# filrg/split_learning

Hardware: AMD Instinct MI355X
Metric: images/sec (whole node) VGG16/CIFAR10 cut=7 (higher is better)
Workload: dtype fp32; 1 GPU; model=VGG16_CIFAR10, global_batch=32, image=3x32x32, cut_layer=7, optimizer=SGD(lr=5e-4, momentum=0.5), control_count=1, mode=serial-recompute, parallelism=split2 x dp1

## Files before the change

split_learning_amd/ops/csrc/bindings.cpp:

```cpp
#include <torch/extension.h>

namespace slk {
at::Tensor matmul_f32(const at::Tensor&, const at::Tensor&, bool, bool,
                      c10::optional<at::Tensor>, bool);
at::Tensor linear_fwd(const at::Tensor&, const at::Tensor&, c10::optional<at::Tensor>);
at::Tensor colsum_f32(const at::Tensor&);
at::Tensor conv2d_wino(const at::Tensor&, const at::Tensor&,
                       c10::optional<at::Tensor>, int, bool);
int conv2d_wino_slabs(int, int, int);
at::Tensor conv2d_wino_bwdw(const at::Tensor&, const at::Tensor&, int);
at::Tensor conv2d_wino_fused(const at::Tensor&, const at::Tensor&,
                             c10::optional<at::Tensor>, int, bool);
at::Tensor conv2d_wino_bwdw_fused(const at::Tensor&, const at::Tensor&, int);
at::Tensor conv2d_fwd(const at::Tensor&, const at::Tensor&, c10::optional<at::Tensor>,
                      int, int);
at::Tensor conv2d_bwd_data(const at::Tensor&, const at::Tensor&, int, int, int, int);
at::Tensor conv2d_bwd_weight(const at::Tensor&, const at::Tensor&, int, int, int, int);
at::Tensor conv2d_bwd_bias(const at::Tensor&);
std::string conv_route(const std::string&, int, int, int, int, int, int, int, int);
std::vector<at::Tensor> bn2d_stats_fused(const at::Tensor&,
                                         c10::optional<at::Tensor>,
                                         c10::optional<at::Tensor>,
                                         c10::optional<at::Tensor>, double, double);
at::Tensor bn2d_fwd(const at::Tensor&, const at::Tensor&, const at::Tensor&,
                    const at::Tensor&, const at::Tensor&, bool);
std::vector<at::Tensor> bn2d_bwd(const at::Tensor&, const at::Tensor&,
                                 const at::Tensor&, const at::Tensor&,
                                 const at::Tensor&, c10::optional<at::Tensor>);
std::vector<at::Tensor> bn2d_bwd_eval(const at::Tensor&, const at::Tensor&,
                                      const at::Tensor&, const at::Tensor&,
                                      const at::Tensor&, c10::optional<at::Tensor>);
std::vector<at::Tensor> bn2d_train_fwd(const at::Tensor&, const at::Tensor&,
                                       const at::Tensor&,
                                       c10::optional<at::Tensor>,
                                       c10::optional<at::Tensor>,
                                       c10::optional<at::Tensor>, double, double,
                                       bool, bool);
std::vector<at::Tensor> bn2d_train_bwd(const at::Tensor&, const at::Tensor&,
                                       const at::Tensor&, const at::Tensor&,
                                       const at::Tensor&, c10::optional<at::Tensor>,
                                       c10::optional<at::Tensor>);
std::vector<at::Tensor> drop_res_ln_fwd(const at::Tensor&, const at::Tensor&,
                                        const at::Tensor&, const at::Tensor&,
                                        double, double, int64_t,
                                        c10::optional<at::Tensor>);
std::vector<at::Tensor> layernorm_fwd(const at::Tensor&, const at::Tensor&,
// ... 36 lines not shown
                double, double, double, double, bool);
at::Tensor make_opt_desc(std::vector<at::Tensor>, std::vector<at::Tensor>,
                         std::vector<at::Tensor>, std::vector<at::Tensor>);
void sgd_step_fused(const at::Tensor&, int64_t, int64_t, double, double, double,
                    bool, bool);
void adamw_step_fused(const at::Tensor&, int64_t, int64_t, int64_t, double, double,
                      double, double, double, bool);
}

PYBIND11_MODULE(TORCH_EXTENSION_NAME, m) {
  m.doc() = "split_learning_amd CDNA4 (gfx950) HIP kernels";
  m.def("matmul_f32", &slk::matmul_f32, py::arg("a"), py::arg("b"),
        py::arg("trans_a") = false, py::arg("trans_b") = false,
        py::arg("out") = py::none(), py::arg("accumulate") = false);
  m.def("linear_fwd", &slk::linear_fwd);
  m.def("colsum_f32", &slk::colsum_f32);
  m.def("conv2d_wino", &slk::conv2d_wino, py::arg("x"), py::arg("w"),
        py::arg("bias") = py::none(), py::arg("pad") = 1,
        py::arg("flip") = false);
  m.def("conv2d_wino_slabs", &slk::conv2d_wino_slabs, py::arg("co"),
        py::arg("ci"), py::arg("tiles"));
  m.def("conv2d_wino_bwdw", &slk::conv2d_wino_bwdw, py::arg("gy"),
        py::arg("x"), py::arg("pad") = 1);
  m.def("conv2d_wino_fused", &slk::conv2d_wino_fused, py::arg("x"),
        py::arg("w"), py::arg("bias") = py::none(), py::arg("pad") = 1,
        py::arg("flip") = false);
  m.def("conv2d_wino_bwdw_fused", &slk::conv2d_wino_bwdw_fused, py::arg("gy"),
        py::arg("x"), py::arg("pad") = 1);
  m.def("conv2d_fwd", &slk::conv2d_fwd, py::arg("x"), py::arg("w"),
        py::arg("bias"), py::arg("stride"), py::arg("pad"));
  m.def("conv2d_bwd_data", &slk::conv2d_bwd_data);
  m.def("conv2d_bwd_weight", &slk::conv2d_bwd_weight, py::arg("gy"), py::arg("x"),
        py::arg("kh"), py::arg("kw"), py::arg("stride"), py::arg("pad"));
  m.def("conv2d_bwd_bias", &slk::conv2d_bwd_bias);
  m.def("conv_route", &slk::conv_route, py::arg("op"), py::arg("B"),
        py::arg("Ci"), py::arg("H"), py::arg("W"), py::arg("Co"), py::arg("K"),
        py::arg("stride"), py::arg("pad"));
  m.def("bn2d_stats_fused", &slk::bn2d_stats_fused);
  m.def("bn2d_fwd", &slk::bn2d_fwd);
  m.def("bn2d_bwd", &slk::bn2d_bwd, py::arg("x"), py::arg("gy"),
        py::arg("gamma"), py::arg("mean"), py::arg("invstd"),
        py::arg("relu_y") = py::none());
  m.def("bn2d_bwd_eval", &slk::bn2d_bwd_eval, py::arg("x"), py::arg("gy"),
        py::arg("gamma"), py::arg("mean"), py::arg("invstd"),
        py::arg("relu_y") = py::none());
  m.def("bn2d_train_fwd", &slk::bn2d_train_fwd, py::arg("x"), py::arg("gamma"),
        py::arg("beta"), py::arg("running_mean"), py::arg("running_var"),
        py::arg("num_batches_tracked"), py::arg("momentum"), py::arg("eps"),
        py::arg("relu") = false, py::arg("pool") = false);
  m.def("bn2d_train_bwd", &slk::bn2d_train_bwd, py::arg("x"), py::arg("gy"),
        py::arg("gamma"), py::arg("mean"), py::arg("invstd"),
        py::arg("relu_y") = py::none(), py::arg("idx") = py::none());
  m.def("drop_res_ln_fwd", &slk::drop_res_ln_fwd, py::arg("x"), py::arg("res"),
        py::arg("gamma"), py::arg("beta"), py::arg("eps"), py::arg("p") = 0.0,
        py::arg("seed") = 0, py::arg("offset") = py::none());
  m.def("layernorm_fwd", &slk::layernorm_fwd);
  m.def("layernorm_bwd", &slk::layernorm_bwd);
  m.def("relu_fwd", &slk::relu_fwd);
  m.def("relu_bwd", &slk::relu_bwd);
  m.def("gelu_fwd", &slk::gelu_fwd);
  m.def("gelu_bwd", &slk::gelu_bwd);
  m.def("tanh_fwd", &slk::tanh_fwd);
  m.def("tanh_bwd", &slk::tanh_bwd);
  m.def("dropout_fwd", &slk::dropout_fwd);
  m.def("dropout_fwd_dev", &slk::dropout_fwd_dev);
  m.def("dropout_bwd", &slk::dropout_bwd);
// ... 25 lines not shown
```

split_learning_amd/ops/csrc/conv2d.hip:

```cpp
#include <tuple>

#include "conv_route.h"
#include "tile_gemm.h"
#include "torch_util.h"

namespace slk {

at::Tensor conv2d_wino(const at::Tensor&, const at::Tensor&,
                       c10::optional<at::Tensor>, int, bool);
at::Tensor conv2d_wino_bwdw(const at::Tensor&, const at::Tensor&, int);
at::Tensor conv2d_wino_fused(const at::Tensor&, const at::Tensor&,
                             c10::optional<at::Tensor>, int, bool);
at::Tensor conv2d_wino_bwdw_fused(const at::Tensor&, const at::Tensor&, int);

static int wino_level() {
  static const int v = [] {
    const char* e = std::getenv("SLK_WINO");
    return e ? atoi(e) : 1;
  }();
  return v;
}

struct ConvGeom {
  int B, Ci, H, W, Co, KH, KW, OH, OW, stride, pad;
  FastDiv d_ohow, d_ow, d_hw, d_w, d_khkw, d_kw;
};

template <int CKH, int CKW, int CS>
struct Geo {
  static constexpr bool fixed = CKH > 0;
  __device__ static int kh_kw(const ConvGeom& g) { return fixed ? CKH * CKW : g.KH * g.KW; }
  __device__ static int stride(const ConvGeom& g) { return fixed ? CS : g.stride; }
  __device__ static void dk(const ConvGeom& g, int k, int& c, int& kh, int& kw) {
    if (fixed) {
      c = k / (CKH * CKW);
      const int r = k - c * (CKH * CKW);
      kh = r / CKW;
      kw = r - kh * CKW;
    } else {
      c = g.d_khkw.div(k);
      const int r = g.d_khkw.mod(k, c);
      kh = g.d_kw.div(r);
      kw = g.d_kw.mod(r, kh);
    }
  }
};
// ... 180 lines not shown
    return {ci * geo.H * geo.W, (short)kh, (short)kw, valid};
  }
  __device__ float loadB(const BCtx& c, const KCtx&, int k, bool kv) const {
    const unsigned b = geo.d_ohow.div(k);
    const unsigned rem = geo.d_ohow.mod(k, b);
    const unsigned oh = geo.d_ow.div(rem);
    const unsigned ow = geo.d_ow.mod(rem, oh);
    const int ih = (int)oh * G::stride(geo) - geo.pad + c.kh;
    const int iw = (int)ow * G::stride(geo) - geo.pad + c.kw;
    const bool in = (unsigned)ih < (unsigned)geo.H && (unsigned)iw < (unsigned)geo.W;
    const int ihc = in ? ih : 0;
    const int iwc = in ? iw : 0;
    const float v = x[(long)b * geo.Ci * geo.H * geo.W + c.ciHW
                      + ihc * geo.W + iwc];
    return sel0(v, c.valid & kv & in);
  }
};

struct AtomicStore {
  float* c;
  int N;
  bool accumulate;
  long slab_stride;
  __device__ void store(int, int m, int n, float v, int ks) const {
    float* p = c + (long)ks * slab_stride + (long)m * N + n;
    if (accumulate) {
      atomicAdd(p, v);
    } else {
      *p = v;
    }
  }
};

__global__ void slab_reduce_kernel(const float* __restrict__ slab, int splits,
                                   float* __restrict__ out, long numel) {
  const long stride = (long)gridDim.x * blockDim.x;
  for (long i = (long)blockIdx.x * blockDim.x + threadIdx.x; i < numel;
       i += stride) {
    float s = 0.f;
    for (int k = 0; k < splits; ++k) s += slab[(long)k * numel + i];
    out[i] = s;
  }
}

void slab_reduce(const float* slab, int splits, float* out, long numel,
                 hipStream_t stream) {
  const int grid = (int)std::min<long>((numel + 255) / 256, 4096);
  hipLaunchKernelGGL(slab_reduce_kernel, dim3(grid), dim3(256), 0, stream,
                     slab, splits, out, numel);
}

static inline int slab_min_splits() {
  static int v = [] {
    const char* e = std::getenv("SLK_SLAB_MIN");
    return e ? atoi(e) : 3;
  }();
  return v < 2 ? 2 : v;
}

static constexpr long SLK_SLAB_MAX_BYTES = 32l << 20;


static ConvShape conv_shape(int B, int Ci, int H, int W, int Co, int KH, int KW,
                            int stride, int pad) {
  return {B, Ci, H, W, Co, KH, KW, stride, pad};
}

static ConvGeom make_geom(const ConvShape& s) {
  ConvGeom g;
  g.B = s.B; g.Ci = s.Ci; g.H = s.H; g.W = s.W; g.Co = s.Co; g.KH = s.KH;
  g.KW = s.KW; g.stride = s.stride; g.pad = s.pad;
  g.OH = s.OH();
  g.OW = s.OW();
  g.d_ohow.init(g.OH * g.OW);
  g.d_ow.init(g.OW);
  g.d_hw.init(g.H * g.W);
  g.d_w.init(g.W);
  g.d_khkw.init(g.KH * g.KW);
  g.d_kw.init(g.KW);
  return g;
}

// ... 124 lines not shown
                                slab_stride};
      });
}

at::Tensor conv2d_bwd_weight(const at::Tensor& gy, const at::Tensor& x, int KH,
                             int KW, int stride, int pad) {
  TORCH_CHECK(gy.is_cuda() && x.is_cuda() && gy.scalar_type() == at::kFloat);
  const ConvShape s = conv_shape(x.size(0), x.size(1), x.size(2), x.size(3),
                                 gy.size(1), KH, KW, stride, pad);
  TORCH_CHECK(s.OH() == gy.size(2) && s.OW() == gy.size(3),
              "bwd-weight geometry mismatch");
  switch (route_bwd_weight(s, wino_level())) {
    case ConvRoute::WinoBwdWFused:
      return conv2d_wino_bwdw_fused(gy, x, pad);
    case ConvRoute::WinoBwdW:
      return conv2d_wino_bwdw(gy, x, pad);
    default:
      break;
  }
  auto gyc = gy.contiguous();
  auto xc = x.contiguous();
  const ConvGeom geo = make_geom(s);
  const int N = geo.Ci * KH * KW;
  const bool fast = (geo.OH * geo.OW) % SLK_BK == 0;
  return direct_gemm<ConvBwdWeightGather>(
      geo, geo.Co, N, geo.B * geo.OH * geo.OW, {geo.Co, geo.Ci, KH, KW},
      gy.options(), gyc.data_ptr<float>(), xc.data_ptr<float>(),
      [&](float* gw, bool accumulate, long slab_stride) {
        return AtomicStore{gw, N, accumulate, slab_stride};
      },
      fast);
}

std::string conv_route(const std::string& op, int B, int Ci, int H, int W,
                       int Co, int K, int stride, int pad) {
  const ConvShape s = conv_shape(B, Ci, H, W, Co, K, K, stride, pad);
  if (op == "fwd") return conv_route_name(route_fwd(s, wino_level()));
  if (op == "bwd_data") return conv_route_name(route_bwd_data(s, wino_level()));
  TORCH_CHECK(op == "bwd_weight", "conv_route: op must be fwd, bwd_data or "
              "bwd_weight, got ", op);
  return conv_route_name(route_bwd_weight(s, wino_level()));
}

__global__ void conv_bias_grad_kernel(const float* __restrict__ gy,
                                      float* __restrict__ slab, int B, int C,
                                      int HW) {
  __shared__ float scratch[16];
  const int c = blockIdx.x;
  const int total = B * HW;
  const int per = (total + gridDim.y - 1) / gridDim.y;
  const int lo = blockIdx.y * per;
  const int hi = min(total, lo + per);
  float acc = 0.f;
  for (int i = lo + threadIdx.x; i < hi; i += blockDim.x) {
    const int b = i / HW;
    const int r = i - b * HW;
    acc += gy[((long)b * C + c) * HW + r];
  }
  float total_s = slk_block_sum(acc, scratch);
  if (threadIdx.x == 0) slab[(long)blockIdx.y * C + c] = total_s;
}

__global__ void conv_bias_finalize_kernel(const float* __restrict__ slab,
                                          int chunks, float* __restrict__ gb,
                                          int C) {
  const int c = blockIdx.x * blockDim.x + threadIdx.x;
// ... 24 lines not shown
```

split_learning_amd/ops/csrc/torch_util.h:

```cpp
#pragma once

#include <torch/extension.h>
#include <ATen/ATen.h>
#include <c10/hip/HIPStream.h>

#include "common.h"

namespace slk {

static inline at::Tensor zeroed(at::IntArrayRef sizes, const at::TensorOptions& opt) {
  auto t = at::empty(sizes, opt);
  slk_zero_async(t.data_ptr<float>(), t.numel(),
                 c10::hip::getCurrentHIPStream().stream());
  return t;
}

static inline int reduce_chunks(long per_channel) {
  long c = per_channel / 4096;
  if (c < 1) c = 1;
  if (c > 16) c = 16;
  return (int)c;
}

void slab_reduce(const float* slab, int splits, float* out, long numel,
                 hipStream_t stream);

}
```

split_learning_amd/ops/csrc/wino.hip:

```cpp
#include "torch_util.h"

namespace slk {

template <bool FLIP>
__device__ __forceinline__ void wino_wt_body(const float* __restrict__ w,
                                             float* __restrict__ U, int Cw0,
                                             int Cw1, int block, int nblocks) {
  const long total = (long)Cw0 * Cw1;
  const long tstride = (long)nblocks * blockDim.x;
  for (long e = (long)block * blockDim.x + threadIdx.x; e < 4 * total;
       e += tstride) {
    const int a = (int)(e & 3);
    const long i = e >> 2;
    const int cols = FLIP ? Cw0 : Cw1;
    const int c = (int)(i % cols);
    const int r = (int)(i / cols);
    const int co = FLIP ? c : r;
    const int ci = FLIP ? r : c;
    float t[3];
    #pragma unroll
    for (int b = 0; b < 3; ++b) {
      const float g0 = w[(((long)co * Cw1 + ci) * 3 + (FLIP ? 2 : 0)) * 3 +
                         (FLIP ? 2 - b : b)];
      const float g1 = w[(((long)co * Cw1 + ci) * 3 + 1) * 3 +
                         (FLIP ? 2 - b : b)];
      const float g2 = w[(((long)co * Cw1 + ci) * 3 + (FLIP ? 0 : 2)) * 3 +
                         (FLIP ? 2 - b : b)];
      t[b] = a == 0 ? g0
           : a == 1 ? 0.5f * (g0 + g1 + g2)
           : a == 2 ? 0.5f * (g0 - g1 + g2)
           : g2;
    }
// ... 288 lines not shown
constexpr int WF_RS = 168;
constexpr int WF_OP = 32 * WF_RS;

__device__ __forceinline__ void wino_kstep_mfma(const float* pa,
                                                const float* pb,
                                                f32x4 (&acc)[16]) {
  const f32x4* a0 = reinterpret_cast<const f32x4*>(pa);
  const f32x4* a1 = reinterpret_cast<const f32x4*>(pa + 4 * WF_KS);
  const f32x4* b0 = reinterpret_cast<const f32x4*>(pb);
  const f32x4* b1 = reinterpret_cast<const f32x4*>(pb + 4 * WF_KS);
  f32x4 ra0 = a0[0], rb0 = b0[0], ra1 = a1[0], rb1 = b1[0];
  #pragma unroll
  for (int g = 0; g < 4; ++g) {
    const f32x4 ca0 = ra0, cb0 = rb0, ca1 = ra1, cb1 = rb1;
    if (g < 3) {
      ra0 = a0[g + 1];
      rb0 = b0[g + 1];
      ra1 = a1[g + 1];
      rb1 = b1[g + 1];
    }
    __builtin_amdgcn_sched_barrier(0);
    #pragma unroll
    for (int j = 0; j < 4; ++j)
      acc[g * 4 + j] = __builtin_amdgcn_mfma_f32_16x16x4f32(
          ca0[j], cb0[j], acc[g * 4 + j], 0, 0, 0);
    #pragma unroll
    for (int j = 0; j < 4; ++j)
      acc[g * 4 + j] = __builtin_amdgcn_mfma_f32_16x16x4f32(
          ca1[j], cb1[j], acc[g * 4 + j], 0, 0, 0);
  }
}

template <bool FLIP>
__global__ __launch_bounds__(256, 3) void wino_fused_kernel(
    const float* __restrict__ x, const float* __restrict__ w,
    const float* __restrict__ bias, float* __restrict__ y, int B, int Ci,
    int H, int W, int Co, int OH, int OW, int tH, int tW, int pad,
    int ci_per, int CW, FastDiv d_thw, FastDiv d_tw) {
  const int ci_begin = blockIdx.z * ci_per;
  const int ci_end = min(Ci, ci_begin + ci_per);
  __shared__ __attribute__((aligned(16))) float Ul[WF_OP];
  __shared__ __attribute__((aligned(16))) float Vl[WF_OP];

  const int T = B * tH * tW;
  const int co0 = blockIdx.y * WF_CO;
  const int t0 = blockIdx.x * WF_T;

  const int tid = threadIdx.x;
  const int lane = tid & 63;
  const int wid = tid >> 6;
  const int wco = (wid >> 1) * 16;
  const int wt = (wid & 1) * 16;
  const int frag_r = lane >> 4;
  const int frag_c = lane & 15;

  f32x4 acc[16];
  #pragma unroll
  for (int f = 0; f < 16; ++f) acc[f] = f32x4{};

  const int v_ci = tid >> 5;
  const int v_t = tid & 31;
  const int tg = t0 + v_t;
  const unsigned vb = d_thw.div((unsigned)tg);
  const unsigned vrem = d_thw.mod((unsigned)tg, vb);
  const unsigned vth = d_tw.div(vrem);
  const unsigned vtw = d_tw.mod(vrem, vth);
  const int ih0 = (int)vth * 2 - pad;
  const int iw0 = (int)vtw * 2 - pad;
  const long xplane = ((long)vb * Ci + v_ci) * H * W;
  const int w_co = tid >> 3;
  const int w_ci = tid & 7;

  float d[4][4];
  f32x4 wq0, wq1;
  float w8;

  auto load_regs = [&](int ci0) {
    const float* xp = x + xplane + (long)ci0 * H * W;
    #pragma unroll
// ... 51 lines not shown
    for (int a = 0; a < 4; ++a) {
      const float* t = tr[a];
      up[a] = f32x4{t[0], 0.5f * (t[0] + t[1] + t[2]),
                    0.5f * (t[0] - t[1] + t[2]), t[2]};
    }
  };

  const float* pa = &Ul[(wco + frag_c) * WF_RS + frag_r * WF_KS];
  const float* pb = &Vl[(wt + frag_c) * WF_RS + frag_r * WF_KS];

  load_regs(ci_begin);
  for (int ci0 = ci_begin; ci0 < ci_end; ci0 += WF_CK) {
    store_stage();
    __syncthreads();
    if (ci0 + WF_CK < ci_end) load_regs(ci0 + WF_CK);
    wino_kstep_mfma(pa, pb, acc);
    __syncthreads();
  }

  #pragma unroll
  for (int i = 0; i < 4; ++i) {
    const int co = co0 + wco + frag_r * 4 + i;
    const int t = t0 + wt + frag_c;
    if (co >= Co || t >= T) continue;
    float m[4][4];
    #pragma unroll
    for (int f = 0; f < 16; ++f) m[f >> 2][f & 3] = acc[f][i];
    float u0[4], u1[4];
    #pragma unroll
    for (int bb = 0; bb < 4; ++bb) {
      u0[bb] = m[0][bb] + m[1][bb] + m[2][bb];
      u1[bb] = m[1][bb] - m[2][bb] - m[3][bb];
    }
    const float bv = (bias != nullptr && blockIdx.z == 0) ? bias[co] : 0.f;
    const unsigned b = d_thw.div((unsigned)t);
    const unsigned rem = d_thw.mod((unsigned)t, b);
    const unsigned th = d_tw.div(rem);
    const unsigned tw = d_tw.mod(rem, th);
    float* yp = y + (long)blockIdx.z * B * Co * OH * OW +
                ((long)b * Co + co) * OH * OW + (long)th * 2 * OW + tw * 2;
    const float o00 = u0[0] + u0[1] + u0[2] + bv;
    const float o01 = u0[1] - u0[2] - u0[3] + bv;
    const float o10 = u1[0] + u1[1] + u1[2] + bv;
    const float o11 = u1[1] - u1[2] - u1[3] + bv;
    yp[0] = o00;
    yp[1] = o01;
    yp[OW] = o10;
    yp[OW + 1] = o11;
  }
}

at::Tensor conv2d_wino_bwdw(const at::Tensor& gy, const at::Tensor& x,
                            int pad) {
  TORCH_CHECK(gy.is_cuda() && x.is_cuda() && gy.dim() == 4 && x.dim() == 4);
  auto gyc = gy.contiguous();
  auto xc = x.contiguous();
  const int B = x.size(0), Ci = x.size(1), H = x.size(2), W = x.size(3);
  const int Co = gy.size(1), OH = gy.size(2), OW = gy.size(3);
  TORCH_CHECK(OH == H + 2 * pad - 2 && OW == W + 2 * pad - 2,
              "wino_bwdw geometry");
  TORCH_CHECK(OH % 2 == 0 && OW % 2 == 0, "wino_bwdw: even output dims only");
  const int tH = OH / 2, tW = OW / 2;
  const int T = B * tH * tW;
  auto stream = c10::hip::getCurrentHIPStream().stream();
  FastDiv d_T, d_thw, d_tw;
  d_T.init(T);
  d_thw.init(tH * tW);
  d_tw.init(tW);

  auto Wg = at::empty({16, Co, T}, x.options());
  auto Vx = at::empty({16, Ci, T}, x.options());
  {
    const long tot = (long)Co * T;
    const int grid = (int)std::min<long>((tot + 255) / 256, 8192);
    hipLaunchKernelGGL(wino_gyA_kernel, dim3(grid), dim3(256), 0, stream,
                       gyc.data_ptr<float>(), Wg.data_ptr<float>(), B, Co, OH,
                       OW, tH, tW, d_T, d_thw, d_tw);
  }
  {
    const long tot = (long)Ci * T;
    const int grid = (int)std::min<long>((tot + 255) / 256, 8192);
    hipLaunchKernelGGL(wino_in_kernel, dim3(grid), dim3(256), 0, stream,
                       xc.data_ptr<float>(), Vx.data_ptr<float>(), B, Ci, H, W,
                       tH, tW, pad, d_T, d_thw, d_tw);
  }
  auto dU = matmul_f32(Wg, Vx, false, true, c10::nullopt, false);
  auto gw = at::empty({Co, Ci, 3, 3}, x.options());
  {
    const long tot = (long)Co * Ci;
    const int grid = (int)std::min<long>((tot + 255) / 256, 4096);
    hipLaunchKernelGGL(wino_gw_kernel, dim3(grid), dim3(256), 0, stream,
                       dU.data_ptr<float>(), gw.data_ptr<float>(), Co, Ci);
  }
  return gw;
}

__global__ __launch_bounds__(256, 2) void wino_bwdw_fused_kernel(
    const float* __restrict__ gy, const float* __restrict__ x,
    float* __restrict__ slab, int B, int Ci, int H, int W, int Co, int OH,
    int OW, int tH, int tW, int pad, int t_per, FastDiv d_thw, FastDiv d_tw) {
  __shared__ __attribute__((aligned(16))) float Gl[WF_OP];
  __shared__ __attribute__((aligned(16))) float Xl[WF_OP];

  const int T = B * tH * tW;
  const int ci0 = blockIdx.y * 32;
  const int co0 = blockIdx.x * 32;
  const int t_begin = blockIdx.z * t_per;
  const int t_end = min(T, t_begin + t_per);

  const int tid = threadIdx.x;
  const int lane = tid & 63;
  const int wid = tid >> 6;
  const int wco = (wid >> 1) * 16;
  const int wci = (wid & 1) * 16;
  const int frag_r = lane >> 4;
  const int frag_c = lane & 15;

  f32x4 acc[16];
  #pragma unroll
  for (int f = 0; f < 16; ++f) acc[f] = f32x4{};

  const int s_ch = tid >> 3;
  const int s_t = tid & 7;

  float gg[2][2];
  float xd[4][4];

  auto load_regs = [&](int t0) {
    const int t = t0 + s_t;
    const int tc = t < T ? t : T - 1;
    const bool tv = t < t_end;
    const unsigned b = d_thw.div((unsigned)tc);
    const unsigned rem = d_thw.mod((unsigned)tc, b);
    const unsigned th = d_tw.div(rem);
    const unsigned tw = d_tw.mod(rem, th);
    {
      const float* gp = gy + ((long)b * Co + co0 + s_ch) * OH * OW
                        + (long)th * 2 * OW + tw * 2;
      gg[0][0] = tv ? gp[0] : 0.f;
      gg[0][1] = tv ? gp[1] : 0.f;
// ... 44 lines not shown
      xp4[a] = f32x4{u[a][0] - u[a][2], u[a][1] + u[a][2],
                     u[a][2] - u[a][1], u[a][1] - u[a][3]};
    }
  };

  const float* pa = &Gl[(wco + frag_c) * WF_RS + frag_r * WF_KS];
  const float* pb = &Xl[(wci + frag_c) * WF_RS + frag_r * WF_KS];

  load_regs(t_begin);
  for (int t0 = t_begin; t0 < t_end; t0 += 8) {
    store_stage();
    __syncthreads();
    if (t0 + 8 < t_end) load_regs(t0 + 8);
    wino_kstep_mfma(pa, pb, acc);
    __syncthreads();
  }

  const long numel = (long)Co * Ci * 9;
  #pragma unroll
  for (int i = 0; i < 4; ++i) {
    const int co = co0 + wco + frag_r * 4 + i;
    const int ci = ci0 + wci + frag_c;
    if (co >= Co || ci >= Ci) continue;
    float u[4][4];
    #pragma unroll
    for (int f = 0; f < 16; ++f) u[f >> 2][f & 3] = acc[f][i];
    float t3[3][4];
    #pragma unroll
    for (int bb = 0; bb < 4; ++bb) {
      t3[0][bb] = u[0][bb] + 0.5f * (u[1][bb] + u[2][bb]);
      t3[1][bb] = 0.5f * (u[1][bb] - u[2][bb]);
      t3[2][bb] = 0.5f * (u[1][bb] + u[2][bb]) + u[3][bb];
    }
    float* gp = slab + (long)blockIdx.z * numel + ((long)co * Ci + ci) * 9;
    #pragma unroll
    for (int r = 0; r < 3; ++r) {
      gp[r * 3 + 0] = t3[r][0] + 0.5f * (t3[r][1] + t3[r][2]);
      gp[r * 3 + 1] = 0.5f * (t3[r][1] - t3[r][2]);
      gp[r * 3 + 2] = 0.5f * (t3[r][1] + t3[r][2]) + t3[r][3];
    }
  }
}

at::Tensor conv2d_wino_bwdw_fused(const at::Tensor& gy, const at::Tensor& x,
                                  int pad) {
  TORCH_CHECK(gy.is_cuda() && x.is_cuda() && gy.dim() == 4 && x.dim() == 4);
  auto gyc = gy.contiguous();
  auto xc = x.contiguous();
  const int B = x.size(0), Ci = x.size(1), H = x.size(2), W = x.size(3);
  const int Co = gy.size(1), OH = gy.size(2), OW = gy.size(3);
  TORCH_CHECK(OH == H + 2 * pad - 2 && OW == W + 2 * pad - 2,
              "wino_bwdw_fused geometry");
  TORCH_CHECK(OH % 2 == 0 && OW % 2 == 0 && Co % 32 == 0 && Ci % 32 == 0,
              "wino_bwdw_fused shape requirements");
  const int tH = OH / 2, tW = OW / 2;
  const int T = B * tH * tW;
  auto stream = c10::hip::getCurrentHIPStream().stream();

  const long base_blocks = (long)(Co / 32) * (Ci / 32);
  int splits = 1;
  if (base_blocks < 256) {
    splits = (int)((256 + base_blocks - 1) / base_blocks);
    const int max_splits = (T + 7) / 8;
    if (splits > max_splits) splits = max_splits;
  }
  int t_per = ((T / splits + 7) / 8) * 8;
  if (t_per < 8) t_per = 8;
  splits = (T + t_per - 1) / t_per;

  auto slab = at::empty({splits, Co, Ci, 3, 3}, x.options());
  FastDiv d_thw, d_tw;
  d_thw.init(tH * tW);
  d_tw.init(tW);
  dim3 grid(Co / 32, Ci / 32, splits);
  hipLaunchKernelGGL(wino_bwdw_fused_kernel, grid, dim3(256), 0, stream,
                     gyc.data_ptr<float>(), xc.data_ptr<float>(),
                     slab.data_ptr<float>(), B, Ci, H, W, Co, OH, OW, tH, tW,
                     pad, t_per, d_thw, d_tw);
  if (splits == 1) {
    return slab.view({Co, Ci, 3, 3});
  }
  auto gw = at::empty({Co, Ci, 3, 3}, x.options());
  slab_reduce(slab.data_ptr<float>(), splits, gw.data_ptr<float>(), gw.numel(),
              stream);
  return gw;
}

at::Tensor conv2d_wino_fused(const at::Tensor& x, const at::Tensor& w,
                             c10::optional<at::Tensor> bias, int pad,
                             bool flip) {
  TORCH_CHECK(x.is_cuda() && x.dim() == 4 && x.scalar_type() == at::kFloat);
  TORCH_CHECK(w.size(2) == 3 && w.size(3) == 3, "wino_fused: 3x3 only");
  auto xc = x.contiguous();
  auto wc = w.contiguous();
  const int B = x.size(0), H = x.size(2), W = x.size(3);
  const int Co = flip ? w.size(1) : w.size(0);
  const int Ci = flip ? w.size(0) : w.size(1);
  TORCH_CHECK(x.size(1) == Ci, "wino_fused: channel mismatch");
  const int OH = H + 2 * pad - 2, OW = W + 2 * pad - 2;
  const int tH = OH / 2, tW = OW / 2;
  const int T = B * tH * tW;
  TORCH_CHECK(Co % 32 == 0 && T % 32 == 0 && Ci % 8 == 0 && OH % 2 == 0
              && OW % 2 == 0, "wino_fused shape requirements");
  auto stream = c10::hip::getCurrentHIPStream().stream();
  const int CW = (int)w.size(1);
  const long base_blocks = (long)(T / 32) * (Co / 32);
  int splits = 1;
  if (base_blocks < 256) {
    splits = (int)((256 + base_blocks - 1) / base_blocks);
    const int max_splits = Ci / WF_CK;
    if (splits > max_splits) splits = max_splits;
  }
  int ci_per = ((Ci / splits + WF_CK - 1) / WF_CK) * WF_CK;
  splits = (Ci + ci_per - 1) / ci_per;

  auto y = at::empty({B, Co, OH, OW}, x.options());
  at::Tensor slab;
  if (splits > 1) slab = at::empty({splits, B, Co, OH, OW}, x.options());
  float* yw = splits > 1 ? slab.data_ptr<float>() : y.data_ptr<float>();
  FastDiv d_thw, d_tw;
  d_thw.init(tH * tW);
  d_tw.init(tW);
  dim3 grid(T / 32, Co / 32, splits);
  if (flip) {
    hipLaunchKernelGGL(wino_fused_kernel<true>, grid, dim3(256), 0, stream,
                       xc.data_ptr<float>(), wc.data_ptr<float>(),
                       bias.has_value() ? bias->data_ptr<float>() : nullptr,
                       yw, B, Ci, H, W, Co, OH, OW, tH, tW,
                       pad, ci_per, CW, d_thw, d_tw);
  } else {
    hipLaunchKernelGGL(wino_fused_kernel<false>, grid, dim3(256), 0, stream,
                       xc.data_ptr<float>(), wc.data_ptr<float>(),
                       bias.has_value() ? bias->data_ptr<float>() : nullptr,
                       yw, B, Ci, H, W, Co, OH, OW, tH, tW,
                       pad, ci_per, CW, d_thw, d_tw);
  }
  if (splits > 1) {
    slab_reduce(slab.data_ptr<float>(), splits, y.data_ptr<float>(), y.numel(),
                stream);
  }
  return y;
}

}
```

split_learning_amd/ops/functional.py:

```python

from __future__ import annotations

import os
from typing import Optional

import torch
import torch.nn.functional as _F
from torch.autograd import Function

from . import native

_LIB_MM_THRESH = float(os.environ.get("SLK_LIB_MM_THRESH", "1e7"))
_LIB_LIN_THRESH = float(os.environ.get("SLK_LIB_LIN_THRESH", "2e7"))


def use_lib_mm(batch, m, n, k) -> bool:
    return 2.0 * batch * m * n * k >= _LIB_MM_THRESH



def _matmul_raw(a, b, trans_a=False, trans_b=False, out=None, accumulate=False):
    return native().matmul_f32(a, b, trans_a, trans_b, out, accumulate)


# ... 57 lines not shown
            gx = gx.reshape(ctx.x_shape)
        if ctx.needs_input_grad[1]:
            gw = _matmul_raw(gys, xs, trans_a=True)
        if ctx.has_bias and ctx.needs_input_grad[2]:
            gb = native().colsum_f32(gys)
        return gx, gw, gb


def linear(x, weight, bias=None):
    rows = x.numel() // x.shape[-1]
    if 2.0 * rows * weight.shape[0] * weight.shape[1] >= _LIB_LIN_THRESH:
        return _F.linear(x, weight, bias)
    return LinearFn.apply(x, weight, bias)



class Conv2dFn(Function):

    @staticmethod
    def forward(ctx, x, weight, bias, stride, padding, bias_grad_zero):
        x = x.contiguous()
        y = native().conv2d_fwd(x, weight, bias, stride, padding)
        ctx.save_for_backward(x, weight)
        ctx.stride = stride
        ctx.padding = padding
        ctx.has_bias = bias is not None
        ctx.bias_grad_zero = bias_grad_zero
        return y

    @staticmethod
    def backward(ctx, gy):
        x, weight = ctx.saved_tensors
        gy = gy.contiguous()
        gx = gw = gb = None
        if ctx.needs_input_grad[0]:
            gx = native().conv2d_bwd_data(gy, weight, ctx.stride, ctx.padding,
                                          x.shape[2], x.shape[3])
        if ctx.needs_input_grad[1]:
            gw = native().conv2d_bwd_weight(gy, x, weight.shape[2], weight.shape[3],
                                            ctx.stride, ctx.padding)
        if ctx.has_bias and ctx.needs_input_grad[2]:
            if ctx.bias_grad_zero:
                gb = None
            else:
                gb = native().conv2d_bwd_bias(gy)
        return gx, gw, gb, None, None, None


def conv2d(x, weight, bias=None, stride=1, padding=0, bias_grad_zero=False):
    return Conv2dFn.apply(x, weight, bias, int(stride), int(padding),
                          bool(bias_grad_zero))



BN_FUSED = os.environ.get("SLK_BN_FUSED", "1") != "0"


class BatchNorm2dFn(Function):
    @staticmethod
    def forward(ctx, x, gamma, beta, running_mean, running_var, training, momentum, eps,
                fuse_relu, num_batches_tracked):
        x = x.contiguous()
        ctx.one_launch = training and BN_FUSED
        if ctx.one_launch:
            y, mean, invstd = native().bn2d_train_fwd(
                x, gamma, beta, running_mean, running_var, num_batches_tracked,
                momentum, eps, fuse_relu, False)
        else:
            if training:
                mean, invstd = native().bn2d_stats_fused(
                    x, running_mean, running_var, num_batches_tracked,
                    momentum, eps)
            else:
# ... 406 lines not shown
```

Baseline: 14780 images/sec.

## Fuse Winograd conv backward-data and backward-weight into one paired launch

```diff
diff --git a/split_learning_amd/ops/csrc/bindings.cpp b/split_learning_amd/ops/csrc/bindings.cpp
--- a/split_learning_amd/ops/csrc/bindings.cpp
+++ b/split_learning_amd/ops/csrc/bindings.cpp
@@ -12,6 +12,12 @@
 at::Tensor conv2d_wino_fused(const at::Tensor&, const at::Tensor&,
                              c10::optional<at::Tensor>, int, bool);
 at::Tensor conv2d_wino_bwdw_fused(const at::Tensor&, const at::Tensor&, int);
+std::tuple<at::Tensor, at::Tensor> conv2d_bwd_pair(const at::Tensor&,
+                                                   const at::Tensor&,
+                                                   const at::Tensor&, int, int);
+std::tuple<int, int, int, int> conv2d_bwd_pair_splits(int, int, int, int, int, int);
+std::tuple<c10::optional<at::Tensor>, c10::optional<at::Tensor>> conv2d_bwd(
+    const at::Tensor&, const at::Tensor&, const at::Tensor&, int, int, bool, bool);
 at::Tensor conv2d_fwd(const at::Tensor&, const at::Tensor&, c10::optional<at::Tensor>,
                       int, int);
 at::Tensor conv2d_bwd_data(const at::Tensor&, const at::Tensor&, int, int, int, int);
@@ -114,6 +120,14 @@
   m.def("conv2d_bwd_data", &slk::conv2d_bwd_data);
   m.def("conv2d_bwd_weight", &slk::conv2d_bwd_weight, py::arg("gy"), py::arg("x"),
         py::arg("kh"), py::arg("kw"), py::arg("stride"), py::arg("pad"));
+  m.def("conv2d_bwd", &slk::conv2d_bwd, py::arg("gy"), py::arg("x"),
+        py::arg("w"), py::arg("stride"), py::arg("pad"), py::arg("need_gx"),
+        py::arg("need_gw"));
+  m.def("conv2d_bwd_pair", &slk::conv2d_bwd_pair, py::arg("gy"), py::arg("x"),
+        py::arg("w"), py::arg("pad") = 1, py::arg("interleave") = -1);
+  m.def("conv2d_bwd_pair_splits", &slk::conv2d_bwd_pair_splits, py::arg("B"),
+        py::arg("Ci"), py::arg("H"), py::arg("W"), py::arg("Co"),
+        py::arg("pad") = 1);
   m.def("conv2d_bwd_bias", &slk::conv2d_bwd_bias);
   m.def("conv_route", &slk::conv_route, py::arg("op"), py::arg("B"),
         py::arg("Ci"), py::arg("H"), py::arg("W"), py::arg("Co"), py::arg("K"),
diff --git a/split_learning_amd/ops/csrc/conv2d.hip b/split_learning_amd/ops/csrc/conv2d.hip
--- a/split_learning_amd/ops/csrc/conv2d.hip
+++ b/split_learning_amd/ops/csrc/conv2d.hip
@@ -12,6 +12,9 @@
 at::Tensor conv2d_wino_fused(const at::Tensor&, const at::Tensor&,
                              c10::optional<at::Tensor>, int, bool);
 at::Tensor conv2d_wino_bwdw_fused(const at::Tensor&, const at::Tensor&, int);
+std::tuple<at::Tensor, at::Tensor> conv2d_bwd_pair(const at::Tensor&,
+                                                   const at::Tensor&,
+                                                   const at::Tensor&, int, int);
 
 static int wino_level() {
   static const int v = [] {
@@ -258,10 +261,13 @@
   }
 };
 
-__global__ void slab_reduce_kernel(const float* __restrict__ slab, int splits,
-                                   float* __restrict__ out, long numel) {
-  const long stride = (long)gridDim.x * blockDim.x;
-  for (long i = (long)blockIdx.x * blockDim.x + threadIdx.x; i < numel;
+__device__ __forceinline__ void slab_reduce_body(const float* __restrict__ slab,
+                                                 int splits,
+                                                 float* __restrict__ out,
+                                                 long numel, int block,
+                                                 int nblocks) {
+  const long stride = (long)nblocks * blockDim.x;
+  for (long i = (long)block * blockDim.x + threadIdx.x; i < numel;
        i += stride) {
     float s = 0.f;
     for (int k = 0; k < splits; ++k) s += slab[(long)k * numel + i];
@@ -269,11 +275,44 @@
   }
 }
 
+__global__ void slab_reduce_kernel(const float* __restrict__ slab, int splits,
+                                   float* __restrict__ out, long numel) {
+  slab_reduce_body(slab, splits, out, numel, blockIdx.x, gridDim.x);
+}
+
+__global__ void slab_reduce_pair_kernel(const float* __restrict__ slab_a,
+                                        int splits_a, float* __restrict__ out_a,
+                                        long numel_a, int blocks_a,
+                                        const float* __restrict__ slab_b,
+                                        int splits_b, float* __restrict__ out_b,
+                                        long numel_b) {
+  if ((int)blockIdx.x < blocks_a) {
+    slab_reduce_body(slab_a, splits_a, out_a, numel_a, blockIdx.x, blocks_a);
+  } else {
+    slab_reduce_body(slab_b, splits_b, out_b, numel_b, blockIdx.x - blocks_a,
+                     gridDim.x - blocks_a);
+  }
+}
+
+static int slab_reduce_grid(long numel) {
+  return (int)std::min<long>((numel + 255) / 256, 4096);
+}
+
 void slab_reduce(const float* slab, int splits, float* out, long numel,
                  hipStream_t stream) {
-  const int grid = (int)std::min<long>((numel + 255) / 256, 4096);
-  hipLaunchKernelGGL(slab_reduce_kernel, dim3(grid), dim3(256), 0, stream,
-                     slab, splits, out, numel);
+  hipLaunchKernelGGL(slab_reduce_kernel, dim3(slab_reduce_grid(numel)),
+                     dim3(256), 0, stream, slab, splits, out, numel);
+}
+
+void slab_reduce_pair(const float* slab_a, int splits_a, float* out_a,
+                      long numel_a, const float* slab_b, int splits_b,
+                      float* out_b, long numel_b, hipStream_t stream) {
+  const int blocks_a = slab_reduce_grid(numel_a);
+  const int blocks_b = slab_reduce_grid(numel_b);
+  if (blocks_a + blocks_b == 0) return;
+  hipLaunchKernelGGL(slab_reduce_pair_kernel, dim3(blocks_a + blocks_b),
+                     dim3(256), 0, stream, slab_a, splits_a, out_a, numel_a,
+                     blocks_a, slab_b, splits_b, out_b, numel_b);
 }
 
 static inline int slab_min_splits() {
@@ -464,6 +503,35 @@
       fast);
 }
 
+static bool conv_bwd_pair_enabled() {
+  static const int v = [] {
+    const char* e = std::getenv("SLK_CONV_BWD_PAIR");
+    return e ? atoi(e) : 1;
+  }();
+  return v != 0;
+}
+
+std::tuple<c10::optional<at::Tensor>, c10::optional<at::Tensor>> conv2d_bwd(
+    const at::Tensor& gy, const at::Tensor& x, const at::Tensor& w, int stride,
+    int pad, bool need_gx, bool need_gw) {
+  TORCH_CHECK(x.dim() == 4 && w.dim() == 4 && gy.dim() == 4);
+  const int H = x.size(2), W = x.size(3), KH = w.size(2), KW = w.size(3);
+  if (need_gx && need_gw && conv_bwd_pair_enabled()) {
+    const ConvShape s = conv_shape(x.size(0), x.size(1), H, W, w.size(0), KH,
+                                   KW, stride, pad);
+    if (s.OH() == gy.size(2) && s.OW() == gy.size(3) &&
+        route_bwd_data(s, wino_level()) == ConvRoute::WinoFused &&
+        route_bwd_weight(s, wino_level()) == ConvRoute::WinoBwdWFused) {
+      auto r = conv2d_bwd_pair(gy, x, w, pad, -1);
+      return {std::get<0>(r), std::get<1>(r)};
+    }
+  }
+  c10::optional<at::Tensor> gx, gw;
+  if (need_gx) gx = conv2d_bwd_data(gy, w, stride, pad, H, W);
+  if (need_gw) gw = conv2d_bwd_weight(gy, x, KH, KW, stride, pad);
+  return {gx, gw};
+}
+
 std::string conv_route(const std::string& op, int B, int Ci, int H, int W,
                        int Co, int K, int stride, int pad) {
   const ConvShape s = conv_shape(B, Ci, H, W, Co, K, K, stride, pad);
diff --git a/split_learning_amd/ops/csrc/torch_util.h b/split_learning_amd/ops/csrc/torch_util.h
--- a/split_learning_amd/ops/csrc/torch_util.h
+++ b/split_learning_amd/ops/csrc/torch_util.h
@@ -24,5 +24,8 @@
 
 void slab_reduce(const float* slab, int splits, float* out, long numel,
                  hipStream_t stream);
+void slab_reduce_pair(const float* slab_a, int splits_a, float* out_a,
+                      long numel_a, const float* slab_b, int splits_b,
+                      float* out_b, long numel_b, hipStream_t stream);
 
 }
diff --git a/split_learning_amd/ops/csrc/wino.hip b/split_learning_amd/ops/csrc/wino.hip
--- a/split_learning_amd/ops/csrc/wino.hip
+++ b/split_learning_amd/ops/csrc/wino.hip
@@ -1,3 +1,5 @@
+#include <tuple>
+
 #include "torch_util.h"
 
 namespace slk {
@@ -352,19 +354,18 @@
 }
 
 template <bool FLIP>
-__global__ __launch_bounds__(256, 3) void wino_fused_kernel(
+__device__ __forceinline__ void wino_fused_body(
+    float (&Ul)[WF_OP], float (&Vl)[WF_OP], unsigned bx, unsigned by, unsigned bz,
     const float* __restrict__ x, const float* __restrict__ w,
     const float* __restrict__ bias, float* __restrict__ y, int B, int Ci,
     int H, int W, int Co, int OH, int OW, int tH, int tW, int pad,
-    int ci_per, int CW, FastDiv d_thw, FastDiv d_tw) {
-  const int ci_begin = blockIdx.z * ci_per;
+    int ci_per, int CW, const FastDiv& d_thw, const FastDiv& d_tw) {
+  const int ci_begin = bz * ci_per;
   const int ci_end = min(Ci, ci_begin + ci_per);
-  __shared__ __attribute__((aligned(16))) float Ul[WF_OP];
-  __shared__ __attribute__((aligned(16))) float Vl[WF_OP];
 
   const int T = B * tH * tW;
-  const int co0 = blockIdx.y * WF_CO;
-  const int t0 = blockIdx.x * WF_T;
+  const int co0 = by * WF_CO;
+  const int t0 = bx * WF_T;
 
   const int tid = threadIdx.x;
   const int lane = tid & 63;
@@ -482,12 +483,12 @@
       u0[bb] = m[0][bb] + m[1][bb] + m[2][bb];
       u1[bb] = m[1][bb] - m[2][bb] - m[3][bb];
     }
-    const float bv = (bias != nullptr && blockIdx.z == 0) ? bias[co] : 0.f;
+    const float bv = (bias != nullptr && bz == 0) ? bias[co] : 0.f;
     const unsigned b = d_thw.div((unsigned)t);
     const unsigned rem = d_thw.mod((unsigned)t, b);
     const unsigned th = d_tw.div(rem);
     const unsigned tw = d_tw.mod(rem, th);
-    float* yp = y + (long)blockIdx.z * B * Co * OH * OW +
+    float* yp = y + (long)bz * B * Co * OH * OW +
                 ((long)b * Co + co) * OH * OW + (long)th * 2 * OW + tw * 2;
     const float o00 = u0[0] + u0[1] + u0[2] + bv;
     const float o01 = u0[1] - u0[2] - u0[3] + bv;
@@ -498,6 +499,19 @@
     yp[OW] = o10;
     yp[OW + 1] = o11;
   }
+}
+
+template <bool FLIP>
+__global__ __launch_bounds__(256, 3) void wino_fused_kernel(
+    const float* __restrict__ x, const float* __restrict__ w,
+    const float* __restrict__ bias, float* __restrict__ y, int B, int Ci,
+    int H, int W, int Co, int OH, int OW, int tH, int tW, int pad,
+    int ci_per, int CW, FastDiv d_thw, FastDiv d_tw) {
+  __shared__ __attribute__((aligned(16))) float Ul[WF_OP];
+  __shared__ __attribute__((aligned(16))) float Vl[WF_OP];
+  wino_fused_body<FLIP>(Ul, Vl, blockIdx.x, blockIdx.y, blockIdx.z, x, w, bias,
+                        y, B, Ci, H, W, Co, OH, OW, tH, tW, pad, ci_per, CW,
+                        d_thw, d_tw);
 }
 
 at::Tensor conv2d_wino_bwdw(const at::Tensor& gy, const at::Tensor& x,
@@ -545,17 +559,16 @@
   return gw;
 }
 
-__global__ __launch_bounds__(256, 2) void wino_bwdw_fused_kernel(
+__device__ __forceinline__ void wino_bwdw_fused_body(
+    float (&Gl)[WF_OP], float (&Xl)[WF_OP], unsigned bx, unsigned by, unsigned bz,
     const float* __restrict__ gy, const float* __restrict__ x,
     float* __restrict__ slab, int B, int Ci, int H, int W, int Co, int OH,
-    int OW, int tH, int tW, int pad, int t_per, FastDiv d_thw, FastDiv d_tw) {
-  __shared__ __attribute__((aligned(16))) float Gl[WF_OP];
-  __shared__ __attribute__((aligned(16))) float Xl[WF_OP];
-
+    int OW, int tH, int tW, int pad, int t_per, const FastDiv& d_thw,
+    const FastDiv& d_tw) {
   const int T = B * tH * tW;
-  const int ci0 = blockIdx.y * 32;
-  const int co0 = blockIdx.x * 32;
-  const int t_begin = blockIdx.z * t_per;
+  const int ci0 = by * 32;
+  const int co0 = bx * 32;
+  const int t_begin = bz * t_per;
   const int t_end = min(T, t_begin + t_per);
 
   const int tid = threadIdx.x;
@@ -666,7 +679,7 @@
       t3[1][bb] = 0.5f * (u[1][bb] - u[2][bb]);
       t3[2][bb] = 0.5f * (u[1][bb] + u[2][bb]) + u[3][bb];
     }
-    float* gp = slab + (long)blockIdx.z * numel + ((long)co * Ci + ci) * 9;
+    float* gp = slab + (long)bz * numel + ((long)co * Ci + ci) * 9;
     #pragma unroll
     for (int r = 0; r < 3; ++r) {
       gp[r * 3 + 0] = t3[r][0] + 0.5f * (t3[r][1] + t3[r][2]);
@@ -674,6 +687,99 @@
       gp[r * 3 + 2] = 0.5f * (t3[r][1] + t3[r][2]) + t3[r][3];
     }
   }
+}
+
+__global__ __launch_bounds__(256, 2) void wino_bwdw_fused_kernel(
+    const float* __restrict__ gy, const float* __restrict__ x,
+    float* __restrict__ slab, int B, int Ci, int H, int W, int Co, int OH,
+    int OW, int tH, int tW, int pad, int t_per, FastDiv d_thw, FastDiv d_tw) {
+  __shared__ __attribute__((aligned(16))) float Gl[WF_OP];
+  __shared__ __attribute__((aligned(16))) float Xl[WF_OP];
+  wino_bwdw_fused_body(Gl, Xl, blockIdx.x, blockIdx.y, blockIdx.z, gy, x, slab,
+                       B, Ci, H, W, Co, OH, OW, tH, tW, pad, t_per, d_thw,
+                       d_tw);
+}
+
+constexpr int WINO_PAIR_INTERLEAVE = 0;
+struct WinoPairData {
+  const float* x; const float* w; float* y;
+  int B, Ci, H, W, Co, OH, OW, tH, tW, pad, ci_per, CW;
+  FastDiv d_thw, d_tw;
+  int gx, gy, n;
+};
+struct WinoPairWeight {
+  const float* gy; const float* x; float* slab;
+  int B, Ci, H, W, Co, OH, OW, tH, tW, pad, t_per;
+  FastDiv d_thw, d_tw;
+  int gx, gy_, n;
+};
+
+__global__ __launch_bounds__(256, 3) void wino_bwd_pair_kernel(
+    WinoPairData d, WinoPairWeight g, int interleave) {
+  __shared__ __attribute__((aligned(16))) float Al[WF_OP];
+  __shared__ __attribute__((aligned(16))) float Bl[WF_OP];
+  const int b = blockIdx.x;
+  bool data;
+  int idx;
+  if (interleave) {
+    const int m = min(d.n, g.n);
+    if (b < 2 * m) {
+      data = (b & 1) == 0;
+      idx = b >> 1;
+    } else {
+      data = d.n > g.n;
+      idx = b - m;
+    }
+  } else {
+    data = b < d.n;
+    idx = data ? b : b - d.n;
+  }
+  if (data) {
+    const int plane = d.gx * d.gy;
+    const int bz = idx / plane;
+    const int r = idx - bz * plane;
+    const int by = r / d.gx;
+    wino_fused_body<true>(Al, Bl, r - by * d.gx, by, bz, d.x, d.w, nullptr,
+                          d.y, d.B, d.Ci, d.H, d.W, d.Co, d.OH, d.OW, d.tH,
+                          d.tW, d.pad, d.ci_per, d.CW, d.d_thw, d.d_tw);
+  } else {
+    const int plane = g.gx * g.gy_;
+    const int bz = idx / plane;
+    const int r = idx - bz * plane;
+    const int by = r / g.gx;
+    wino_bwdw_fused_body(Al, Bl, r - by * g.gx, by, bz, g.gy, g.x, g.slab,
+                         g.B, g.Ci, g.H, g.W, g.Co, g.OH, g.OW, g.tH, g.tW,
+                         g.pad, g.t_per, g.d_thw, g.d_tw);
+  }
+}
+
+struct WinoSplit { int splits, per; };
+
+static WinoSplit wino_fused_split(int Co, int Ci, int T) {
+  const long base_blocks = (long)(T / 32) * (Co / 32);
+  int splits = 1;
+  if (base_blocks < 256) {
+    splits = (int)((256 + base_blocks - 1) / base_blocks);
+    const int max_splits = Ci / WF_CK;
+    if (splits > max_splits) splits = max_splits;
+  }
+  const int ci_per = ((Ci / splits + WF_CK - 1) / WF_CK) * WF_CK;
+  splits = (Ci + ci_per - 1) / ci_per;
+  return {splits, ci_per};
+}
+
+static WinoSplit wino_bwdw_split(int Co, int Ci, int T) {
+  const long base_blocks = (long)(Co / 32) * (Ci / 32);
+  int splits = 1;
+  if (base_blocks < 256) {
+    splits = (int)((256 + base_blocks - 1) / base_blocks);
+    const int max_splits = (T + 7) / 8;
+    if (splits > max_splits) splits = max_splits;
+  }
+  int t_per = ((T / splits + 7) / 8) * 8;
+  if (t_per < 8) t_per = 8;
+  splits = (T + t_per - 1) / t_per;
+  return {splits, t_per};
 }
 
 at::Tensor conv2d_wino_bwdw_fused(const at::Tensor& gy, const at::Tensor& x,
@@ -691,16 +797,8 @@
   const int T = B * tH * tW;
   auto stream = c10::hip::getCurrentHIPStream().stream();
 
-  const long base_blocks = (long)(Co / 32) * (Ci / 32);
-  int splits = 1;
-  if (base_blocks < 256) {
-    splits = (int)((256 + base_blocks - 1) / base_blocks);
-    const int max_splits = (T + 7) / 8;
-    if (splits > max_splits) splits = max_splits;
-  }
-  int t_per = ((T / splits + 7) / 8) * 8;
-  if (t_per < 8) t_per = 8;
-  splits = (T + t_per - 1) / t_per;
+  const WinoSplit sp = wino_bwdw_split(Co, Ci, T);
+  const int splits = sp.splits;
 
   auto slab = at::empty({splits, Co, Ci, 3, 3}, x.options());
   FastDiv d_thw, d_tw;
@@ -710,7 +808,7 @@
   hipLaunchKernelGGL(wino_bwdw_fused_kernel, grid, dim3(256), 0, stream,
                      gyc.data_ptr<float>(), xc.data_ptr<float>(),
                      slab.data_ptr<float>(), B, Ci, H, W, Co, OH, OW, tH, tW,
-                     pad, t_per, d_thw, d_tw);
+                     pad, sp.per, d_thw, d_tw);
   if (splits == 1) {
     return slab.view({Co, Ci, 3, 3});
   }
@@ -738,15 +836,8 @@
               && OW % 2 == 0, "wino_fused shape requirements");
   auto stream = c10::hip::getCurrentHIPStream().stream();
   const int CW = (int)w.size(1);
-  const long base_blocks = (long)(T / 32) * (Co / 32);
-  int splits = 1;
-  if (base_blocks < 256) {
-    splits = (int)((256 + base_blocks - 1) / base_blocks);
-    const int max_splits = Ci / WF_CK;
-    if (splits > max_splits) splits = max_splits;
-  }
-  int ci_per = ((Ci / splits + WF_CK - 1) / WF_CK) * WF_CK;
-  splits = (Ci + ci_per - 1) / ci_per;
+  const WinoSplit sp = wino_fused_split(Co, Ci, T);
+  const int splits = sp.splits, ci_per = sp.per;
 
   auto y = at::empty({B, Co, OH, OW}, x.options());
   at::Tensor slab;
@@ -776,4 +867,76 @@
   return y;
 }
 
-}
+std::tuple<int, int, int, int> conv2d_bwd_pair_splits(int B, int Ci, int H,
+                                                      int W, int Co, int pad) {
+  const int OH = H + 2 * pad - 2, OW = W + 2 * pad - 2;
+  const WinoSplit ds = wino_fused_split(Ci, Co, B * (H / 2) * (W / 2));
+  const WinoSplit ws = wino_bwdw_split(Co, Ci, B * (OH / 2) * (OW / 2));
+  return {ds.splits, ds.per, ws.splits, ws.per};
+}
+
+std::tuple<at::Tensor, at::Tensor> conv2d_bwd_pair(const at::Tensor& gy,
+                                                   const at::Tensor& x,
+                                                   const at::Tensor& w, int pad,
+                                                   int interleave) {
+  TORCH_CHECK(gy.is_cuda() && x.is_cuda() && w.is_cuda() && gy.dim() == 4 &&
+              x.dim() == 4 && w.dim() == 4 && gy.scalar_type() == at::kFloat);
+  TORCH_CHECK(w.size(2) == 3 && w.size(3) == 3, "bwd_pair: 3x3 only");
+  auto gyc = gy.contiguous();
+  auto xc = x.contiguous();
+  auto wc = w.contiguous();
+  const int B = x.size(0), Ci = x.size(1), H = x.size(2), W = x.size(3);
+  const int Co = gy.size(1), OH = gy.size(2), OW = gy.size(3);
+  TORCH_CHECK(gy.size(0) == B && w.size(0) == Co && w.size(1) == Ci &&
+              OH == H + 2 * pad - 2 && OW == W + 2 * pad - 2 && pad <= 2,
+              "bwd_pair geometry");
+  const int dtH = H / 2, dtW = W / 2, dT = B * dtH * dtW;
+  const int wtH = OH / 2, wtW = OW / 2, wT = B * wtH * wtW;
+  TORCH_CHECK(H % 2 == 0 && W % 2 == 0 && OH % 2 == 0 && OW % 2 == 0 &&
+              Ci % 32 == 0 && Co % 32 == 0 && dT % 32 == 0,
+              "bwd_pair shape requirements");
+  auto stream = c10::hip::getCurrentHIPStream().stream();
+  const WinoSplit ds = wino_fused_split(Ci, Co, dT);
+  const WinoSplit ws = wino_bwdw_split(Co, Ci, wT);
+
+  auto gx = at::empty({B, Ci, H, W}, x.options());
+  at::Tensor gx_slab;
+  if (ds.splits > 1) gx_slab = at::empty({ds.splits, B, Ci, H, W}, x.options());
+  auto gw_slab = at::empty({ws.splits, Co, Ci, 3, 3}, x.options());
+
+  WinoPairData d;
+  d.x = gyc.data_ptr<float>();
+  d.w = wc.data_ptr<float>();
+  d.y = ds.splits > 1 ? gx_slab.data_ptr<float>() : gx.data_ptr<float>();
+  d.B = B; d.Ci = Co; d.H = OH; d.W = OW; d.Co = Ci; d.OH = H; d.OW = W;
+  d.tH = dtH; d.tW = dtW; d.pad = 2 - pad; d.ci_per = ds.per; d.CW = Ci;
+  d.d_thw.init(dtH * dtW);
+  d.d_tw.init(dtW);
+  d.gx = dT / 32; d.gy = Ci / 32; d.n = d.gx * d.gy * ds.splits;
+  WinoPairWeight g;
+  g.gy = gyc.data_ptr<float>();
+  g.x = xc.data_ptr<float>();
+  g.slab = gw_slab.data_ptr<float>();
+  g.B = B; g.Ci = Ci; g.H = H; g.W = W; g.Co = Co; g.OH = OH; g.OW = OW;
+  g.tH = wtH; g.tW = wtW; g.pad = pad; g.t_per = ws.per;
+  g.d_thw.init(wtH * wtW);
+  g.d_tw.init(wtW);
+  g.gx = Co / 32; g.gy_ = Ci / 32; g.n = g.gx * g.gy_ * ws.splits;
+  if (interleave < 0) interleave = WINO_PAIR_INTERLEAVE;
+  hipLaunchKernelGGL(wino_bwd_pair_kernel, dim3(d.n + g.n), dim3(256), 0,
+                     stream, d, g, interleave);
+
+  at::Tensor gw = ws.splits > 1 ? at::empty({Co, Ci, 3, 3}, x.options())
+                                : gw_slab.view({Co, Ci, 3, 3});
+  if (ds.splits > 1 || ws.splits > 1) {
+    slab_reduce_pair(ds.splits > 1 ? gx_slab.data_ptr<float>() : nullptr,
+                     ds.splits, gx.data_ptr<float>(),
+                     ds.splits > 1 ? gx.numel() : 0,
+                     ws.splits > 1 ? gw_slab.data_ptr<float>() : nullptr,
+                     ws.splits, gw.data_ptr<float>(),
+                     ws.splits > 1 ? gw.numel() : 0, stream);
+  }
+  return {gx, gw};
+}
+
+}
diff --git a/split_learning_amd/ops/functional.py b/split_learning_amd/ops/functional.py
--- a/split_learning_amd/ops/functional.py
+++ b/split_learning_amd/ops/functional.py
@@ -113,13 +113,10 @@
     def backward(ctx, gy):
         x, weight = ctx.saved_tensors
         gy = gy.contiguous()
-        gx = gw = gb = None
-        if ctx.needs_input_grad[0]:
-            gx = native().conv2d_bwd_data(gy, weight, ctx.stride, ctx.padding,
-                                          x.shape[2], x.shape[3])
-        if ctx.needs_input_grad[1]:
-            gw = native().conv2d_bwd_weight(gy, x, weight.shape[2], weight.shape[3],
-                                            ctx.stride, ctx.padding)
+        gb = None
+        gx, gw = native().conv2d_bwd(gy, x, weight, ctx.stride, ctx.padding,
+                                     ctx.needs_input_grad[0],
+                                     ctx.needs_input_grad[1])
         if ctx.has_bias and ctx.needs_input_grad[2]:
             if ctx.bias_grad_zero:
                 gb = None
```

Result: faster. 15620 images/sec, median of 6 (+5.7%).
